# joeyz0z/ConZIC

Measured on AMD Instinct MI355X. Metric: captions/sec (L=10, K=200, seq order), higher is better.
Workload: dtype bf16

## Files before the change

conzic_amd/csrc/engine.hip:

```cpp
#include <algorithm>
#include <map>
#include <string>
#include <vector>
#include <cmath>
#include <cstddef>
#include <cstring>

#include "../../include/conzic_hip.h"
#include "kernels.h"
#include "bridge_hash.h"

namespace czc {
thread_local char g_err[512] = {0};
thread_local int g_gemm_family = 0;
}
using namespace czc;

namespace {

struct Tensor {
  float* p = nullptr;
  std::vector<int64_t> shape;
  size_t numel = 0;
};
// ... 70 lines not shown
  float* d_img_n = nullptr; int img_B = 0;
  float logit_scale_exp = 1.f;
  int* h_totals = nullptr;
  int last_BT = 0, last_B = 0, last_T = 0;
  int bert_prune = 1;
  int bert_pruned_idx = -1;
  const int32_t* bert_pruned_rows = nullptr;
  int bert_fuse_splitk_ln = 1;
  int share_prefix = 1;
  int dedup = 1;
  float* d_staged = nullptr; int staged_cap = 0, staged_n = 0;
  int pack_branches = 1;
  int pool_last_layer = 1;
  int share_layer0 = 1;
  int pool_last_qkv = 1;
  int fuse_ln = 1;
  int resid16 = 1;
  int fold_ln = 1;
  int prof = 0;
  std::map<std::string, ProfKind> pk;
  int64_t stat_clip_rows = 0, stat_clip_seqs = 0, stat_bert_rows = 0, stat_steps = 0;
  int64_t stat_refine_rows = 0, stat_refine_seqs = 0;
  int64_t stat_dedup_seqs = 0;
  czc_control_fn ctl_fn = nullptr; void* ctl_user = nullptr;
  int32_t* h_ctl_ids = nullptr; float* h_ctl_scores = nullptr; size_t h_ctl_cap = 0;
  int memo = 0;
  int64_t stat_memo_hits = 0, stat_memo_images = 0;
  int memo_rows = 0;
  int64_t stat_memo_row_hits = 0, stat_memo_row_steps = 0;
  int32_t* h_memo_list = nullptr; size_t h_memo_list_cap = 0;
// ... 128 lines not shown
    E_HIP(hipMemcpyAsync(l.qkv_b + 2 * H, vb, (size_t)H * 4, hipMemcpyDeviceToDevice, e->st));
    E_CHECK(need(e, o + ".weight", (size_t)H * H, &t)); E_CHECK(to_act(e, prec, t, (size_t)H * H, &l.o_w));
    E_CHECK(need(e, o + ".bias", H, &l.o_b));
    E_CHECK(need(e, ln1 + ".weight", H, &l.ln1_g)); E_CHECK(need(e, ln1 + ".bias", H, &l.ln1_b));
    E_CHECK(need(e, fc1 + ".weight", (size_t)I * H, &t)); E_CHECK(to_act(e, prec, t, (size_t)I * H, &l.fc1_w));
    E_CHECK(need(e, fc1 + ".bias", I, &l.fc1_b));
    E_CHECK(need(e, fc2 + ".weight", (size_t)H * I, &t)); E_CHECK(to_act(e, prec, t, (size_t)H * I, &l.fc2_w));
    E_CHECK(need(e, fc2 + ".bias", H, &l.fc2_b));
    E_CHECK(need(e, ln2 + ".weight", H, &l.ln2_g)); E_CHECK(need(e, ln2 + ".bias", H, &l.ln2_b));
  }
  return 0;
}

int gemm_ex(czc_engine* e, int prec, const char* kind, const GemmArgs& g) {
  ProfScope ps(e, kind, 2.0 * g.M * (double)g.N * g.K);
  E_CHECK(launch_gemm(prec, g, e->st));
  return 0;
}

int gemm(czc_engine* e, int prec, const char* kind, const void* A, int lda, const void* W, int ldw, const float* bias,
         const float* resid, int ldr, void* out_act, float* out_f32, int ldc, int M, int N, int K, int act) {
  GemmArgs g;
  g.A = A; g.lda = lda; g.W = W; g.ldw = ldw; g.bias = bias; g.resid = resid; g.ldr = ldr;
  g.out_act = out_act; g.out_f32 = out_f32; g.ldc = ldc; g.M = M; g.N = N; g.K = K; g.act = act;
  return gemm_ex(e, prec, kind, g);
}

int gemm_x16(czc_engine* e, int prec, const char* kind, const void* A, int lda, const void* W, const float* bias, void* x16, int M,
             int N, int K, float* part = nullptr, long part_ld = 0) {
  GemmArgs g;
  g.A = A; g.lda = lda; g.W = W; g.ldw = K; g.bias = bias; g.resid = (const float*)x16; g.ldr = N;
  g.out_act = nullptr; g.out_f32 = (float*)x16; g.ldc = N; g.M = M; g.N = N; g.K = K; g.act = ACT_NONE; g.x16 = 1;
  g.row_part = part; g.part_ld = part_ld;
// ... 30 lines not shown
  TowerPlan tp; const int* pool_idx = nullptr; int n_pool = 0; bool r16 = false; const float* ln_stat0 = nullptr; Layer0Rows l0;
};

int clip_stack(czc_engine* e, const StackDesc& d, float* x, float** pooled = nullptr) {
  const int P = d.P, M = d.M, H = d.H, I = d.I, heads = d.heads, max_keys = d.max_keys, n_pool = d.n_pool;
  const float eps = d.eps; const bool r16 = d.r16; const char* gk = d.gk; const size_t esz = prec_bytes(P);
  const SegTable& tab = d.tab; const TowerPlan& tp = d.tp; const Layer0Rows& l0 = d.l0; std::vector<LayerW>& L = *d.L;
  void *y, *qkv, *ctx, *hbuf;
  E_CHECK(ensure(e, "cs_y", (size_t)M * H * esz, &y));
  E_CHECK(ensure(e, "cs_qkv", (size_t)M * 3 * H * esz, &qkv));
  E_CHECK(ensure(e, "cs_ctx", (size_t)M * H * esz, &ctx));
  E_CHECK(ensure(e, "cs_h", (size_t)M * I * esz, &hbuf));
  const float scale = 1.0f / sqrtf(64.0f);
  const bool text = !strcmp(gk, "gemm_clip_text") || !strcmp(gk, "gemm_clip_refine");
  const char *ak = text ? "attention_clip_text" : "attention", *rk = text ? "rowops_clip_text" : "rowops";
  const double attn_flops = 4.0 * H * tp.pairs;
  const bool rowln = !r16 && prec_is_half(P) && e->fuse_ln && H == 512 && M >= g_rowln_min_m && I % 32 == 0;
  const bool fold = r16 && e->fold_ln && !L.empty() && L[0].qkv_wf && d.ln_stat0;
  float *part = nullptr, *stat = nullptr;
  if (fold) E_CHECK(ensure(e, "cs_part", (size_t)(H / 32) * M * 8, (void**)&part));
  if (fold) E_CHECK(ensure(e, "cs_stat", (size_t)M * 8 + 256, (void**)&stat));
  auto finalize = [&](int rows, int N, bool always = false) -> int {
    if (!always && gemm_wreg_stats_in_kernel(rows, N)) return 0;
    ProfScope ps(e, rk, 0);
    return launch_ln_finalize(part, M, H / 32, rows, eps, stat, e->st);
  };
  auto folded_gemm = [&](const void* Ax, const void* Wf, const float* bf, const float* st_, void* out, int rows, int N, int act, int ldc = 0) -> int {
    GemmArgs g;
    g.A = Ax; g.lda = H; g.W = Wf; g.ldw = H; g.bias = bf; g.resid = nullptr; g.ldr = 0; g.out_act = out; g.out_f32 = nullptr; g.ldc = ldc ? ldc : N;
    g.M = rows; g.N = N; g.K = H; g.act = act;
// ... 1009 lines not shown
    snprintf(czc::g_err, sizeof(czc::g_err), "czc_create: unknown precision");
    return CZC_ERR_ARG;
  }
  int ndev = 0;
  if (hipGetDeviceCount(&ndev) != hipSuccess || ndev <= 0) {
    snprintf(czc::g_err, sizeof(czc::g_err), "czc_create: no HIP device visible (the engine has no CPU fallback)");
    return CZC_ERR_HIP;
  }
  if (device_id < 0 || device_id >= ndev) {
    snprintf(czc::g_err, sizeof(czc::g_err), "czc_create: device %d out of range", device_id);
    return CZC_ERR_ARG;
  }
  czc_engine* e = new czc_engine();
  e->cfg = *cfg;
  e->dev = device_id;
  e->refine = cfg->precision == CZC_PREC_REFINE;
  e->pc = cfg->precision == CZC_PREC_F32 ? PREC_F32
          : (cfg->precision == CZC_PREC_SPLIT ? PREC_F16X3
             : ((cfg->precision == CZC_PREC_FP16 || e->refine) ? PREC_F16 : PREC_BF16));
  e->pb = cfg->precision == CZC_PREC_ALL_BF16 ? PREC_BF16
                                              : (cfg->precision == CZC_PREC_F32 ? PREC_F32 : PREC_F16X3);
  e->pv = e->refine ? (int)PREC_F16X3 : e->pc;
  e->esz = prec_bytes(e->pc);
  e->eb = prec_bytes(e->pb);
  if (hipSetDevice(device_id) != hipSuccess || hipStreamCreate(&e->st) != hipSuccess ||
      hipHostMalloc((void**)&e->h_totals, 256) != hipSuccess) {
    snprintf(czc::g_err, sizeof(czc::g_err), "czc_create: stream/host allocation failed");
    delete e;
    return CZC_ERR_HIP;
  }
// ... 30 lines not shown
int czc_replicate(czc_engine* p, czc_engine** out) {
  if (!p || !out) return CZC_ERR_ARG;
  if (!p->finalized) return fail(p, CZC_ERR_STATE, "czc_replicate: czc_finalize_weights first%s");
  czc_engine* e = new czc_engine();
  e->cfg = p->cfg; e->dev = p->dev; e->finalized = true; e->shares_weights = true;
  e->esz = p->esz; e->pb = p->pb; e->pc = p->pc; e->pv = p->pv; e->eb = p->eb;
  e->refine = p->refine; e->refine_theta_x = p->refine_theta_x; e->refine_samples = p->refine_samples; e->refine_samples_step = p->refine_samples_step;
  e->refine_guard_dev = p->refine_guard_dev; e->refine_gate_delta = p->refine_gate_delta; e->refine_theta_gen = p->refine_theta_gen;
  e->refine_rows16 = p->refine_rows16; e->refine_rows16_factor = p->refine_rows16_factor;
  e->memo = p->memo; e->memo_rows = p->memo_rows; e->fluency_chunk = p->fluency_chunk; e->regions_chunk = p->regions_chunk;
  e->w = p->w; e->bert = p->bert; e->ctext = p->ctext; e->cvis = p->cvis; e->ctext_x = p->ctext_x;
  e->mlm_dense_w = p->mlm_dense_w; e->decoder_w = p->decoder_w; e->tproj_w = p->tproj_w; e->vproj_w = p->vproj_w;
  e->patch_w = p->patch_w; e->tproj_wx = p->tproj_wx;
  e->logit_scale_exp = p->logit_scale_exp;
  e->share_prefix = p->share_prefix; e->dedup = p->dedup; e->pack_branches = p->pack_branches; e->pool_last_layer = p->pool_last_layer; e->pool_last_qkv = p->pool_last_qkv; e->share_layer0 = p->share_layer0;
  e->fuse_ln = p->fuse_ln; e->bert_prune = p->bert_prune; e->bert_fuse_splitk_ln = p->bert_fuse_splitk_ln; e->resid16 = p->resid16; e->fold_ln = p->fold_ln;
  memset(&e->bd, 0, sizeof(e->bd));
  if (hipSetDevice(e->dev) != hipSuccess || hipStreamCreate(&e->st) != hipSuccess ||
      hipHostMalloc((void**)&e->h_totals, 256) != hipSuccess) {
    e->w.clear();
    delete e;
    return fail(p, CZC_ERR_HIP, "czc_replicate: stream/host allocation failed%s");
  }
  *out = e;
  return CZC_OK;
}

int czc_load_tensor(czc_engine* e, const char* name, int dtype, int ndim, const int64_t* shape, const void* src) {
  if (e && e->shares_weights) return fail(e, CZC_ERR_STATE, "czc_load_tensor: a replica shares its parent's weights%s");
  if (!e || !name || !src || ndim < 0 || ndim > 8) return CZC_ERR_ARG;
// ... 1281 lines not shown
  e->ctl_fn = fn;
  e->ctl_user = fn ? user : nullptr;
  return CZC_OK;
}

int czc_set_option(czc_engine* e, const char* name, int value) {
  if (!e || !name) return CZC_ERR_ARG;
  if (!strcmp(name, "share_prefix")) { e->share_prefix = value ? 1 : 0; return CZC_OK; }
  if (!strcmp(name, "dedup")) { e->dedup = value ? 1 : 0; return CZC_OK; }
  if (!strcmp(name, "bert_prune")) { e->bert_prune = value ? 1 : 0; return CZC_OK; }
  if (!strcmp(name, "bert_fuse_splitk_ln")) { e->bert_fuse_splitk_ln = value ? 1 : 0; return CZC_OK; }
  if (!strcmp(name, "pack_branches")) { e->pack_branches = value ? 1 : 0; return CZC_OK; }
  if (!strcmp(name, "pool_last_layer")) { e->pool_last_layer = value ? 1 : 0; return CZC_OK; }
  if (!strcmp(name, "share_layer0")) { e->share_layer0 = value ? 1 : 0; return CZC_OK; }
  if (!strcmp(name, "pool_last_qkv")) { e->pool_last_qkv = value ? 1 : 0; return CZC_OK; }
  if (!strcmp(name, "fuse_ln")) { e->fuse_ln = value; return CZC_OK; }
  const auto fold_ready = [&]() -> int {
    if (e->finalized && wants_folded_ln(e) && (e->ctext.empty() || !e->ctext[0].qkv_wf))
      return fail(e, CZC_ERR_STATE, "option %s: this engine was finalized without the folded-LayerNorm operands (set it before czc_finalize_weights)", name);
    return CZC_OK;
  };
  if (!strcmp(name, "resid16")) { const int old = e->resid16; e->resid16 = value < 0 ? 0 : value; const int rc = fold_ready(); if (rc) e->resid16 = old; return rc; }
  if (!strcmp(name, "fold_ln")) { const int old = e->fold_ln; e->fold_ln = value ? 1 : 0; const int rc = fold_ready(); if (rc) e->fold_ln = old; return rc; }
  if (!strcmp(name, "refine_samples")) { e->refine_samples = value < 0 ? 0 : value; return CZC_OK; }
  if (!strcmp(name, "refine_samples_step")) { e->refine_samples_step = value < 0 ? 0 : value; return CZC_OK; }
  if (!strcmp(name, "refine_theta_x1000")) { e->refine_theta_x = (float)value / 1000.f; return CZC_OK; }
  if (!strcmp(name, "refine_theta_gen_x1000")) { e->refine_theta_gen = (float)value / 1000.f; return CZC_OK; }
  if (!strcmp(name, "refine_guard_x1e6")) { e->refine_guard_dev = (float)value * 1e-6f; return CZC_OK; }
  if (!strcmp(name, "refine_gate_x1e6")) { e->refine_gate_delta = value < 0 ? 0.f : (float)value * 1e-6f; return CZC_OK; }
  if (!strcmp(name, "refine_rows16")) { const int old = e->refine_rows16; e->refine_rows16 = value ? 1 : 0; const int rc = fold_ready(); if (rc) e->refine_rows16 = old; return rc; }
// ... 12 lines not shown
  if (!strcmp(name, "regions_chunk")) {
    if (value < 1 || value > CZC_MAX_REGIONS) return fail(e, CZC_ERR_ARG, "option %s: 1..1024", name);
    e->regions_chunk = value;
    return CZC_OK;
  }
  if (!strcmp(name, "refine_rows16_x1000")) { e->refine_rows16_factor = value < 1000 ? 1.f : (float)value / 1000.f; return CZC_OK; }
  return fail(e, CZC_ERR_ARG, "unknown option %s", name);
}

int czc_get_option(czc_engine* e, const char* name, int* value) {
  if (!e || !name || !value) return CZC_ERR_ARG;
  const bool r16 = e->refine && e->refine_rows16 && e->cfg.clip_hidden == 512;
  const float f16x = r16 ? e->refine_rows16_factor : 1.f;
  struct { const char* n; int v; } tab[] = {
      {"share_prefix", e->share_prefix}, {"bert_prune", e->bert_prune}, {"pack_branches", e->pack_branches},
      {"dedup", e->dedup}, {"pool_last_layer", e->pool_last_layer}, {"pool_last_qkv", e->pool_last_qkv}, {"share_layer0", e->share_layer0}, {"bert_fuse_splitk_ln", e->bert_fuse_splitk_ln}, {"fuse_ln", e->fuse_ln}, {"resid16", e->resid16}, {"fold_ln", e->fold_ln},
      {"refine_samples", e->refine_samples}, {"refine_samples_step", e->refine_samples_step}, {"refine_theta_x1000", (int)lrintf(e->refine_theta_x * 1000.f)},
      {"refine_theta_gen_x1000", (int)lrintf(e->refine_theta_gen * 1000.f)},
      {"refine_guard_x1e6", (int)lrintf(e->refine_guard_dev * 1e6f)}, {"refine_gate_x1e6", (int)lrintf(e->refine_gate_delta * 1e6f)},
      {"refine_rows16", e->refine_rows16}, {"memo", e->memo}, {"memo_rows", e->memo_rows}, {"index_groups", e->index_groups}, {"fluency_chunk", e->fluency_chunk}, {"regions_chunk", e->regions_chunk}, {"refine_rows16_x1000", (int)lrintf(e->refine_rows16_factor * 1000.f)},
      {"refine_guard_generate_x1e6", (int)lrintf(e->refine_guard_dev * f16x * 1e6f)},
      {"refine_gate_generate_x1e6", (int)lrintf(e->refine_gate_delta * f16x * 1e6f)},
      {"has_folded_ln_weights", !e->ctext.empty() && e->ctext[0].qkv_wf ? 1 : 0},
  };
  for (auto& t : tab) if (!strcmp(name, t.n)) { *value = t.v; return CZC_OK; }
  return fail(e, CZC_ERR_ARG, "unknown option %s", name);
}

int czc_sync(czc_engine* e) {
  if (!e) return CZC_ERR_ARG;
  E_HIP(hipSetDevice(e->dev));
// ... 162 lines not shown
```

conzic_amd/csrc/gemm256.hip:

```cpp
#include <type_traits>

#include "kernels.h"

namespace czc {

namespace {

constexpr int TM = 256, TN = 256;

template <int ACT>
__device__ __forceinline__ float act_fn(float v) {
  if (ACT == ACT_QUICK_GELU) return v * __builtin_amdgcn_rcpf(1.0f + __builtin_amdgcn_exp2f(-2.4554669595930156f * v));
  return v;
}

__device__ __forceinline__ void tile_of(int t, int tiles_m, int tiles_n, int& tm, int& tn) {
  const int nt = tiles_m * tiles_n;
  const int xcd = t & 7, q = nt >> 3, r = nt & 7;
  const int base = (xcd < r) ? xcd * (q + 1) : r * (q + 1) + (xcd - r) * q;
  const int lin = base + (t >> 3);
  tm = lin / tiles_n;
  tn = lin - tm * tiles_n;
}

// ... 337 lines not shown
          unsigned char* dst = oa + ((long)row * g.ldc + c8) * 4;
          *(h8*)dst = hh;
          *(h8*)(dst + 16) = ll;
        }
      }
    }
  }
}

__device__ __forceinline__ int tile_count(int tiles_m, int tiles_n) {
  const int grid = gridDim.x, wg = blockIdx.x, nt = tiles_m * tiles_n;
  return wg < nt ? (nt - 1 - wg) / grid + 1 : 0;
}
__device__ __forceinline__ void tile_at(int i, int tiles_m, int tiles_n, int& tm, int& tn) {
  tile_of(blockIdx.x + i * gridDim.x, tiles_m, tiles_n, tm, tn);
}

__device__ __forceinline__ void start_stagger(int stagger, int nt, int share) {
  if (!stagger) return;
  const int b = (int)blockIdx.x, tau = stagger & 255, bonus = stagger >> 8;
  const int rem = nt % (int)gridDim.x;
  unsigned long long dt = (unsigned long long)(((b >> 3) / share) & 7) * tau;
  if (rem && b >= rem) dt += bonus;
  dt *= 100ull;
  const unsigned long long t0 = __builtin_amdgcn_s_memrealtime();
  while (__builtin_amdgcn_s_memrealtime() - t0 < dt) __builtin_amdgcn_s_sleep(8);
}

constexpr int QROWB = 64;
constexpr int QA_BYTES = TM * QROWB;
// ... 113 lines not shown
      a0 = CZC_RA(1, 2);
      CZC_MM(c0, a1, 1, 0); CZC_MM(c1, a1, 1, 1);
      a1 = CZC_RA(1, 3);
      CZC_MM(c0, a0, 2, 0); CZC_MM(c1, a0, 2, 1);
      CZC_MM(c0, a1, 3, 0); CZC_MM(c1, a1, 3, 1);
#undef CZC_RA
#undef CZC_RB
#undef CZC_MM
    }
    tile_epilogue<ACT, OUT_F32, HT>(g, acc, smem + QS * QSTAGE + wave * 4096, m0, n0, wm, wn, lane);
  }
}



template <int ACT, bool OUT_F32, bool F16 = false, bool X16 = false>
__global__ __launch_bounds__(512) void gemm256x_kernel(GemmArgs g, int tiles_m, int tiles_n, int stagger) {
  using HT = std::conditional_t<F16, f16_t, bf16_t>;
  extern __shared__ __attribute__((aligned(16))) unsigned char smem[];
  const int tid = threadIdx.x;
  const int lane = tid & 63;
  const int wave = __builtin_amdgcn_readfirstlane(tid >> 6);
  const int nk = g.K >> 5;
  const int lda_b = g.lda * 2, ldw_b = g.ldw * 2;
  start_stagger(stagger, tiles_m * tiles_n, tiles_n);
  const int my_tiles = tile_count(tiles_m, tiles_n);
  const int total = my_tiles * nk;

  const unsigned lds0 = __builtin_amdgcn_readfirstlane(
      (unsigned)(unsigned long long)(__attribute__((address_space(3))) unsigned char*)smem);
  const int rbase = wave * 32 + (lane >> 2);
  const int cq = ((lane & 3) ^ ((lane >> 4) & 3)) << 4;
  const int a0 = rbase * lda_b + cq, w0 = rbase * ldw_b + cq;
  const int a16 = 16 * lda_b, w16 = 16 * ldw_b;
  u32x4_t rsA, rsW;
  rsA.x = rsA.y = rsA.z = 0; rsA.w = 0x00020000u;
  rsW = rsA;
  int is = 0, is_ti = 0, is_kt = 0;
  auto issue_rebase = [&]() {
    int tm, tn;
    tile_at(is_ti, tiles_m, tiles_n, tm, tn);
    const int m0 = tm * TM, n0 = tn * TN;
    const unsigned long long pa = (unsigned long long)g.A + (unsigned long long)m0 * lda_b;
    const unsigned long long pw = (unsigned long long)g.W + (unsigned long long)n0 * ldw_b;
    rsA.x = (unsigned)pa; rsA.y = (unsigned)(pa >> 32) & 0xffffu; rsA.z = (unsigned)(min(TM, g.M - m0) * lda_b);
    rsW.x = (unsigned)pw; rsW.y = (unsigned)(pw >> 32) & 0xffffu; rsW.z = (unsigned)(min(TN, g.N - n0) * ldw_b);
  };
  auto issue_next = [&]() {
    const unsigned dstA = lds0 + (is & (QS - 1)) * QSTAGE + wave * (32 * QROWB);
    const unsigned dstW = dstA + QA_BYTES;
    const unsigned so = is_kt * QROWB;
    unsigned keep;
    asm volatile(
        "s_mov_b32 %0, m0\n\t"
        "s_mov_b32 m0, %1\n\ts_nop 0\n\tbuffer_load_dwordx4 %3, %7, %9 offen lds\n\t"
        "s_add_u32 m0, m0, 0x400\n\ts_nop 0\n\tbuffer_load_dwordx4 %4, %7, %9 offen lds\n\t"
// ... 18 lines not shown
    for (int s = 0; s < AHEAD && s < total; ++s) issue_next();
    {
      const int later = (total < AHEAD ? total : AHEAD) - 1;
      if (later >= 2) asm volatile("s_waitcnt vmcnt(8)" ::: "memory");
      else if (later == 1) asm volatile("s_waitcnt vmcnt(4)" ::: "memory");
      else asm volatile("s_waitcnt vmcnt(0)" ::: "memory");
    }
    __builtin_amdgcn_s_barrier();
    asm volatile("" ::: "memory");

    const int wn = wave & 3;
    const int half = lane >> 5;
    const int arow = GRP * 128 + (lane & 31);
    const int brow = wn * 64 + (lane & 31);
    int step = 0;
    const int steady_end = total - 3;
    for (int ti = 0; ti < my_tiles; ++ti) {
      int tm, tn;
      tile_at(ti, tiles_m, tiles_n, tm, tn);
      const int m0 = tm * TM, n0 = tn * TN;
      f32x16_t acc[4][2];
#pragma unroll
      for (int i = 0; i < 4; ++i)
#pragma unroll
        for (int j = 0; j < 2; ++j)
#pragma unroll
          for (int r = 0; r < 16; ++r) acc[i][j][r] = 0.f;
      if (GRP) {
        __builtin_amdgcn_s_barrier();
        asm volatile("" ::: "memory");
      }
      auto kstep = [&](auto steady_c) __attribute__((always_inline)) {
        constexpr bool STEADY = decltype(steady_c)::value;
        const unsigned char* sA = smem + (step & (QS - 1)) * QSTAGE;
        const unsigned char* sB = sA + QA_BYTES;
        if (STEADY || step + AHEAD < total) issue_next();
        uint4 fa[2][4], fb[2][2];
#pragma unroll
        for (int ks = 0; ks < 2; ++ks) {
#pragma unroll
          for (int j = 0; j < 2; ++j) fb[ks][j] = *(const uint4*)(sB + swzq(brow + 32 * j, 2 * ks + half));
#pragma unroll
          for (int i = 0; i < 4; ++i) fa[ks][i] = *(const uint4*)(sA + swzq(arow + 32 * i, 2 * ks + half));
        }
        if (GRP) {
          if (STEADY || step + 3 < total) asm volatile("s_waitcnt vmcnt(8)" ::: "memory");
          else if (step + 2 < total) asm volatile("s_waitcnt vmcnt(4)" ::: "memory");
          else asm volatile("s_waitcnt vmcnt(0)" ::: "memory");
        }
        __builtin_amdgcn_sched_barrier(0);
        __builtin_amdgcn_s_barrier();
        asm volatile("" ::: "memory");
        __builtin_amdgcn_s_setprio(1);
#pragma unroll
        for (int ks = 0; ks < 2; ++ks)
#pragma unroll
          for (int i = 0; i < 4; ++i)
#pragma unroll
            for (int j = 0; j < 2; ++j) acc[i][j] = Half<HT>::mfma(fb[ks][j], fa[ks][i], acc[i][j]);
        __builtin_amdgcn_s_setprio(0);
        __builtin_amdgcn_sched_barrier(0);
        if (!GRP) {
          if (STEADY || step + 2 < total) asm volatile("s_waitcnt vmcnt(4)" ::: "memory");
          else asm volatile("s_waitcnt vmcnt(0)" ::: "memory");
        }
        __builtin_amdgcn_s_barrier();
        asm volatile("" ::: "memory");
      };
      int kt = 0;
      for (; kt < nk && step < steady_end; ++kt, ++step) kstep(std::true_type());
      for (; kt < nk; ++kt, ++step) kstep(std::false_type());
      if (!GRP) {
        __builtin_amdgcn_s_barrier();
        asm volatile("" ::: "memory");
      }
      unsigned char* patch = smem + QS * QSTAGE + wave * 4096;
      if constexpr (X16) {
        tile_epilogue_x16_asm<2>(g, acc, patch, m0, n0, GRP, wn * 64, lane);
      } else if constexpr (OUT_F32 && ACT == ACT_NONE) {
        if (g.resid && g.out_f32 && !g.out_act) tile_epilogue_f32_asm<2>(g, acc, patch, m0, n0, GRP, wn * 64, lane);
        else tile_epilogue<ACT, OUT_F32, HT>(g, acc, patch, m0, n0, GRP, wn, lane);
      } else {
        tile_epilogue<ACT, OUT_F32, HT>(g, acc, patch, m0, n0, GRP, wn, lane);
      }
    }
  };
  if (wave >> 2) run(std::integral_constant<int, 1>());
  else run(std::integral_constant<int, 0>());
}

template <int ACT, bool OUT_F32>
__global__ __launch_bounds__(768) void gemm256sq_kernel(GemmArgs g, int tiles_m, int tiles_n) {
  extern __shared__ __attribute__((aligned(16))) unsigned char smem[];
  const int tid = threadIdx.x;
  const int lane = tid & 63;
  const int wave = __builtin_amdgcn_readfirstlane(tid >> 6);
  const int nk = g.K >> 4;
  const int lda_b = g.lda * 4, ldw_b = g.ldw * 4;
  const int my_tiles = tile_count(tiles_m, tiles_n);
// ... 418 lines not shown
}

int launch_gemm256(const GemmArgs& g, hipStream_t st) {
  constexpr int shp = QS * QSTAGE + 8 * 4096;
  static PerDeviceInit per_dev;
  const LaunchInit init = per_dev.get([](LaunchInit&) -> int {
#define CZC_ATTR(K_) CZC_HIP_CHECK(hipFuncSetAttribute((const void*)K_, hipFuncAttributeMaxDynamicSharedMemorySize, shp))
#define CZC_ATTR4(K_) CZC_ATTR((K_<ACT_NONE, false, false>)); CZC_ATTR((K_<ACT_NONE, true, false>)); \
                      CZC_ATTR((K_<ACT_QUICK_GELU, false, false>)); CZC_ATTR((K_<ACT_QUICK_GELU, true, false>)); \
                      CZC_ATTR((K_<ACT_NONE, false, true>)); CZC_ATTR((K_<ACT_NONE, true, true>)); \
                      CZC_ATTR((K_<ACT_QUICK_GELU, false, true>)); CZC_ATTR((K_<ACT_QUICK_GELU, true, true>))
    CZC_ATTR4(gemm256q_kernel);
    CZC_ATTR4(gemm256x_kernel);
    CZC_ATTR((gemm256x_kernel<ACT_NONE, true, false, true>));
    CZC_ATTR((gemm256x_kernel<ACT_NONE, true, true, true>));
#undef CZC_ATTR4
#undef CZC_ATTR
    return 0;
  });
  if (init.rc) return launch_init_failed("gemm256");
  const int n_cu = init.n_cu;
  const int tiles_m = cdiv(g.M, TM), tiles_n = cdiv(g.N, TN);
  const bool f32 = g.out_f32 != nullptr || g.resid != nullptr;
  dim3 gq(tiles_m * tiles_n < n_cu ? tiles_m * tiles_n : n_cu);
  const bool pp = g_use_gemm256 == 5 || (g_use_gemm256 != 3 && f32);
  g_gemm_family = (g.x16 || pp) ? GF_RING_PINGPONG : GF_RING_LOADER;
#define CZC_GO(K_, A_, F_, H_, T_, ...) hipLaunchKernelGGL((K_<A_, F_, H_>), gq, dim3(T_), shp, st, g, tiles_m, tiles_n, ##__VA_ARGS__)
#define CZC_DISPATCH(K_, T_, ...)                                                                                          \
  do {                                                                                                                     \
    if (g.f16) {                                                                                                           \
      if (g.act == ACT_QUICK_GELU) { if (f32) CZC_GO(K_, ACT_QUICK_GELU, true, true, T_, ##__VA_ARGS__); else CZC_GO(K_, ACT_QUICK_GELU, false, true, T_, ##__VA_ARGS__); } \
      else { if (f32) CZC_GO(K_, ACT_NONE, true, true, T_, ##__VA_ARGS__); else CZC_GO(K_, ACT_NONE, false, true, T_, ##__VA_ARGS__); }                               \
    } else {                                                                                                               \
      if (g.act == ACT_QUICK_GELU) { if (f32) CZC_GO(K_, ACT_QUICK_GELU, true, false, T_, ##__VA_ARGS__); else CZC_GO(K_, ACT_QUICK_GELU, false, false, T_, ##__VA_ARGS__); } \
      else { if (f32) CZC_GO(K_, ACT_NONE, true, false, T_, ##__VA_ARGS__); else CZC_GO(K_, ACT_NONE, false, false, T_, ##__VA_ARGS__); }                             \
    }                                                                                                                      \
  } while (0)
  const int stagger256 = (f32 && tiles_m * tiles_n / (int)gq.x >= 4) ? (2 | 32 << 8) : 0;
  if (g.x16) {
    if (g.f16) hipLaunchKernelGGL((gemm256x_kernel<ACT_NONE, true, true, true>), gq, dim3(512), shp, st, g, tiles_m, tiles_n, stagger256);
    else hipLaunchKernelGGL((gemm256x_kernel<ACT_NONE, true, false, true>), gq, dim3(512), shp, st, g, tiles_m, tiles_n, stagger256);
  } else if (pp) CZC_DISPATCH(gemm256x_kernel, 512, stagger256);
  else CZC_DISPATCH(gemm256q_kernel, 768);
#undef CZC_DISPATCH
#undef CZC_GO
  CZC_HIP_CHECK(hipGetLastError());
  return 0;
}

int g_use_gemm256s = 1;
int g_gemm256s_min_m = 16384;

bool gemm256s_eligible(const GemmArgs& g) {
  return g_use_gemm256s && g.M >= g_gemm256s_min_m && g.N % 8 == 0 && g.K % 32 == 0 && g.ldc % 8 == 0 && g.lda % 8 == 0 && g.ldw % 8 == 0 &&
// ... 31 lines not shown
```

conzic_amd/csrc/kernels.h:

```cpp
#pragma once
#include <vector>

#include "common.h"

namespace czc {

struct GemmArgs {
  const void* A = nullptr; int lda = 0;
  const void* W = nullptr; int ldw = 0;
  const float* bias = nullptr;
  const float* resid = nullptr; int ldr = 0;
  void* out_act = nullptr; float* out_f32 = nullptr; int ldc = 0;
  int M = 0, N = 0, K = 0;
  int act = 0;
  int f16 = 0;
  int x16 = 0;
  float* row_part = nullptr;
  long part_ld = 0;
  const float* ln_stat = nullptr;
  const float* ln_part = nullptr;
  long ln_part_ld = 0;
  const float* ln_gamma = nullptr;
  const float* ln_beta = nullptr;
  float ln_eps = 0.f;
  struct SplitkPending* splitk_pending = nullptr;
};
struct SplitkPending { const float* slabs = nullptr; int nslab = 0; long slab_stride = 0; int ld = 0; };
enum GemmFamily {
  GF_NONE = 0, GF_TILED_VEC = 1, GF_TILED_SCALAR = 2, GF_SPLITK = 3, GF_SKINNY = 4, GF_RING_LOADER = 5, GF_RING_PINGPONG = 6,
  GF_RING_SPLIT = 7, GF_WREG = 8, GF_WREG_LNF = 9, GF_WREG_RESID = 10, GF_ROWLN = 11
};
int launch_gemm(int prec, const GemmArgs& g, hipStream_t st);
bool gemm256_eligible(const GemmArgs& g);
int launch_gemm256(const GemmArgs& g, hipStream_t st);
extern int g_use_gemm256;
bool gemm256s_eligible(const GemmArgs& g);
int launch_gemm256s(const GemmArgs& g, hipStream_t st);
extern int g_use_gemm256s, g_gemm256s_min_m;
bool gemm_rowln_eligible(const GemmArgs& g);
int launch_gemm_rowln(const GemmArgs& g, hipStream_t st);
// ... 218 lines not shown
int launch_refine_finish(const int* own_off, const int* own_len, const int* count, const int* count_off, const int* kr_dev, int B, int K,
                         int* pre_off, int* eos_idx, hipStream_t st);

int launch_normalize_split(const float* src, long n, int D, split_t* dst, int* bad, int bad_stride, hipStream_t st);
int index_scan_groups(int n, int D, int k, int groups);
int launch_index_search(const split_t* index, int n, int D, const split_t* queries, int Q, int k, int G,
                        unsigned long long* part, int* out_ids, float* out_cos, hipStream_t st);

int fluency_expand_tables(int R, int seed_len, int Lmax, const int32_t* len_of_row, int32_t* row_of_seq, int32_t* col_of_seq);
int launch_expand_mask_rows(const int* rows, int T, const int* row_of_seq, const int* col_of_seq, int N, int mask_id, int* ids_out,
                            int* target, int* gen_rows, hipStream_t st);
int launch_logprob_target(const float* logits, int N, int V, const int* target, float temperature, const int* out_idx, float* logp,
                          int* rank, int* nonfinite, hipStream_t st);
int launch_pll_sum(const float* logp, int R, int Lmax, const int* len_of_row, float* pll, hipStream_t st);

constexpr int HOOKS_ABI = 0x060e;
struct Hooks {
  char* (*err_buf)();
  decltype(&launch_gemm) gemm;
  decltype(&launch_gemm_rowln) gemm_rowln;
  decltype(&launch_layernorm) layernorm;
  decltype(&launch_convert) convert;
  decltype(&launch_act_to_f32) act_to_f32;
  decltype(&launch_attention) attention;
  decltype(&launch_attention_shared) attention_shared;
  decltype(&launch_attention_shared_split) attention_shared_split;
  decltype(&launch_softmax_mask_topk) softmax_mask_topk;
  decltype(&launch_bridge_precompute) bridge_precompute;
  decltype(&launch_bridge) bridge;
  decltype(&launch_l2_normalize) l2_normalize;
  decltype(&launch_combine) combine;
// ... 59 lines not shown
```

conzic_amd/native.py:

```python
from __future__ import annotations

import ctypes as C
import os
from typing import Optional

_HERE = os.path.dirname(os.path.abspath(__file__))
LIB_PATH = os.environ.get("CZC_LIB_PATH") or os.path.join(_HERE, "lib", "libconzic_hip.so")
HEADER_PATH = os.path.join(os.path.dirname(_HERE), "include", "conzic_hip.h")
TEST_LIB_PATH = os.environ.get("CZC_TEST_LIB_PATH") or (LIB_PATH[:-3] + "_test.so" if LIB_PATH.endswith(".so")
                                                        else os.path.join(os.path.dirname(LIB_PATH), "libconzic_hip_test.so"))
TEST_HEADER_PATH = os.path.join(os.path.dirname(_HERE), "include", "conzic_hip_test.h")

PREC_BF16 = 0
PREC_F32 = 1
PREC_ALL_BF16 = 2
PREC_SPLIT = 3
PREC_FP16 = 4
PREC_REFINE = 5
CLIP_MAX_LEN = 77
MAX_BERT_LEN = 64
MAX_VOCAB_SETS = 4096
MAX_TOPK = 1024
MAX_RIVALS = 16
MAX_REGIONS = 1024
# ... 114 lines not shown
    "czc_memo_stats": (_I, [_P, C.POINTER(C.c_int64), C.POINTER(C.c_int64)]),
    "czc_memo_rows_stats": (_I, [_P, C.POINTER(C.c_int64), C.POINTER(C.c_int64)]),
}
PRIVATE_SIGNATURES = {"czc_internal_hooks": (_P, [_I])}


class GemmLayout(C.Structure):
    _fields_ = ([(n, C.c_int32) for n in ("precision", "form", "M", "N", "K", "act", "lda", "ldw", "ldc", "ldr", "c0", "flags",
                                          "part_ld")] + [("eps", C.c_float)] +
                [(n, C.c_void_p) for n in ("A", "W", "bias", "resid", "gamma", "beta", "ln_part", "out_f32", "out_act", "part_out")])


TEST_SIGNATURES = {
    "czc_test_gemm": (_I, [_I, _I, _I, _I, _P, _P, _P, _P, _I, _P]),
    "czc_test_gemm_x16": (_I, [_I, _I, _I, _I, _P, _P, _P, _P, _P, _P]),
    "czc_test_ln_fold_gemm": (_I, [_I, _I, _I, _P, _P, _P, _P, _P, _P, C.c_float, _I, _P, _P]),
    "czc_test_layernorm_x16": (_I, [_I, _I, _P, _P, _P, C.c_float, _P]),
    "czc_test_gemm_rowln": (_I, [_I, _I, _I, _P, _P, _P, _P, _P, _P, C.c_float, _P, _P]),
    "czc_bench_gemm": (_I, [_I, _I, _I, _I, _I, _I, _I, _I, C.POINTER(C.c_double)]),
    "czc_test_set_option": (_I, [C.c_char_p, _I]),
    "czc_test_layernorm": (_I, [_I, _I, _I, _P, _P, _P, C.c_float, _P]),
    "czc_test_attention": (_I, [_I, _I, _P, _I, _I, C.c_float, _P, _P]),
    "czc_test_attention_plan": (_I, [_I, _I, _I, _I, _I, C.c_float, _P, _P, _I, _P, _P]),
    "czc_test_attention_pooled": (_I, [_I, _I, _I, _I, C.c_float, _P, _P, _P, _P, _P, _P]),
    "czc_test_attention_seq": (_I, [_I, _I, _P, _I, _I, _I, _I, C.c_float, _P, _P]),
    "czc_test_attention_mapped": (_I, [_I, _I, _I, _I, C.c_float, _P, _P, _P, _I, _P, _P]),
    "czc_test_layer0_plan": (_I, [_I, _I, _P, _P, _I, _P, _P, _P, _P, _I, _P, _I, _P]),
    "czc_test_text_tower": (_I, [_P, _I, _I, _P, _P, _P, _P]),
    "czc_test_topk": (_I, [_I, _I, _I, _P, _P, C.c_float, _I, _I, _P, _P, _P]),
    "czc_test_bridge": (_I, [C.POINTER(BridgeTables), C.POINTER(Config), _I, _I, _P, _P, _P]),
# ... 80 lines not shown
```

Measured before the change: 83.40.

## Add dynamic atomic tile scheduling to persistent 256x GEMM for text tower

Adds a DYN variant of the persistent gemm256x kernel in which blocks pull output tiles from per-slot atomic counters instead of a static strided assignment. The next tile index is prefetched with an in-loop global atomic issued by wave 0. Counters come from a pooled device buffer that is reset once per CLIP text/refine stack pass. The aim is to balance load across CUs when the tile count exceeds the grid. In exchange it adds atomics, extra LDS traffic and a memset per pass, and it relies on inline asm for exec-masking and waitcnt handling.

```diff
diff --git a/conzic_amd/csrc/engine.hip b/conzic_amd/csrc/engine.hip
--- a/conzic_amd/csrc/engine.hip
+++ b/conzic_amd/csrc/engine.hip
@@ -5,6 +5,7 @@
 #include <cmath>
 #include <cstddef>
 #include <cstring>
+#include <cstdlib>
 
 #include "../../include/conzic_hip.h"
 #include "kernels.h"
@@ -108,6 +109,9 @@
   int pool_last_layer = 1;
   int share_layer0 = 1;
   int pool_last_qkv = 1;
+  int dyn_tiles = 1;
+  DynCounters dyn;
+  bool dyn_pass = false;
   int fuse_ln = 1;
   int resid16 = 1;
   int fold_ln = 1;
@@ -266,9 +270,34 @@
 
 int gemm_ex(czc_engine* e, int prec, const char* kind, const GemmArgs& g) {
   ProfScope ps(e, kind, 2.0 * g.M * (double)g.N * g.K);
+  if (e->dyn_pass && !g.dyn_ctr) {
+    GemmArgs gd = g;
+    gd.dyn_ctr = e->dyn.take();
+    E_CHECK(launch_gemm(prec, gd, e->st));
+    return 0;
+  }
   E_CHECK(launch_gemm(prec, g, e->st));
   return 0;
 }
+
+constexpr int DYN_POOL_BLOCKS = 256;
+struct DynPass {
+  czc_engine* e;
+  explicit DynPass(czc_engine* e_) : e(e_) {}
+  int open() {
+    if (!e->dyn_tiles) return 0;
+    void* p;
+    E_CHECK(ensure(e, "cs_dyn", (size_t)DYN_POOL_BLOCKS * DYN_CTR_INTS * 4, &p));
+    if (e->dyn.base != (int*)p) {
+      E_HIP(hipMemsetAsync(p, 0, (size_t)DYN_POOL_BLOCKS * DYN_CTR_INTS * 4, e->st));
+      e->dyn.base = (int*)p; e->dyn.n_blocks = DYN_POOL_BLOCKS; e->dyn.next = 0;
+    }
+    E_HIP(e->dyn.reset(e->st));
+    e->dyn_pass = true;
+    return 0;
+  }
+  ~DynPass() { e->dyn_pass = false; }
+};
 
 int gemm(czc_engine* e, int prec, const char* kind, const void* A, int lda, const void* W, int ldw, const float* bias,
          const float* resid, int ldr, void* out_act, float* out_f32, int ldc, int M, int N, int K, int act) {
@@ -329,6 +358,8 @@
   const float scale = 1.0f / sqrtf(64.0f);
   const bool text = !strcmp(gk, "gemm_clip_text") || !strcmp(gk, "gemm_clip_refine");
   const char *ak = text ? "attention_clip_text" : "attention", *rk = text ? "rowops_clip_text" : "rowops";
+  DynPass dyn_pass(e);
+  if (text) E_CHECK(dyn_pass.open());
   const double attn_flops = 4.0 * H * tp.pairs;
   const bool rowln = !r16 && prec_is_half(P) && e->fuse_ln && H == 512 && M >= g_rowln_min_m && I % 32 == 0;
   const bool fold = r16 && e->fold_ln && !L.empty() && L[0].qkv_wf && d.ln_stat0;
@@ -1368,6 +1399,7 @@
   czc_engine* e = new czc_engine();
   e->cfg = *cfg;
   e->dev = device_id;
+  if (const char* v = getenv("CZC_DYN_TILES")) e->dyn_tiles = atoi(v) ? 1 : 0;
   e->refine = cfg->precision == CZC_PREC_REFINE;
   e->pc = cfg->precision == CZC_PREC_F32 ? PREC_F32
           : (cfg->precision == CZC_PREC_SPLIT ? PREC_F16X3
@@ -1428,6 +1460,7 @@
   e->patch_w = p->patch_w; e->tproj_wx = p->tproj_wx;
   e->logit_scale_exp = p->logit_scale_exp;
   e->share_prefix = p->share_prefix; e->dedup = p->dedup; e->pack_branches = p->pack_branches; e->pool_last_layer = p->pool_last_layer; e->pool_last_qkv = p->pool_last_qkv; e->share_layer0 = p->share_layer0;
+  e->dyn_tiles = p->dyn_tiles;
   e->fuse_ln = p->fuse_ln; e->bert_prune = p->bert_prune; e->bert_fuse_splitk_ln = p->bert_fuse_splitk_ln; e->resid16 = p->resid16; e->fold_ln = p->fold_ln;
   memset(&e->bd, 0, sizeof(e->bd));
   if (hipSetDevice(e->dev) != hipSuccess || hipStreamCreate(&e->st) != hipSuccess ||
@@ -2739,6 +2772,7 @@
   if (!strcmp(name, "pool_last_layer")) { e->pool_last_layer = value ? 1 : 0; return CZC_OK; }
   if (!strcmp(name, "share_layer0")) { e->share_layer0 = value ? 1 : 0; return CZC_OK; }
   if (!strcmp(name, "pool_last_qkv")) { e->pool_last_qkv = value ? 1 : 0; return CZC_OK; }
+  if (!strcmp(name, "dyn_tiles")) { e->dyn_tiles = value ? 1 : 0; return CZC_OK; }
   if (!strcmp(name, "fuse_ln")) { e->fuse_ln = value; return CZC_OK; }
   const auto fold_ready = [&]() -> int {
     if (e->finalized && wants_folded_ln(e) && (e->ctext.empty() || !e->ctext[0].qkv_wf))
@@ -2781,7 +2815,7 @@
   const float f16x = r16 ? e->refine_rows16_factor : 1.f;
   struct { const char* n; int v; } tab[] = {
       {"share_prefix", e->share_prefix}, {"bert_prune", e->bert_prune}, {"pack_branches", e->pack_branches},
-      {"dedup", e->dedup}, {"pool_last_layer", e->pool_last_layer}, {"pool_last_qkv", e->pool_last_qkv}, {"share_layer0", e->share_layer0}, {"bert_fuse_splitk_ln", e->bert_fuse_splitk_ln}, {"fuse_ln", e->fuse_ln}, {"resid16", e->resid16}, {"fold_ln", e->fold_ln},
+      {"dedup", e->dedup}, {"pool_last_layer", e->pool_last_layer}, {"pool_last_qkv", e->pool_last_qkv}, {"share_layer0", e->share_layer0}, {"bert_fuse_splitk_ln", e->bert_fuse_splitk_ln}, {"fuse_ln", e->fuse_ln}, {"dyn_tiles", e->dyn_tiles}, {"resid16", e->resid16}, {"fold_ln", e->fold_ln},
       {"refine_samples", e->refine_samples}, {"refine_samples_step", e->refine_samples_step}, {"refine_theta_x1000", (int)lrintf(e->refine_theta_x * 1000.f)},
       {"refine_theta_gen_x1000", (int)lrintf(e->refine_theta_gen * 1000.f)},
       {"refine_guard_x1e6", (int)lrintf(e->refine_guard_dev * 1e6f)}, {"refine_gate_x1e6", (int)lrintf(e->refine_gate_delta * 1e6f)},
diff --git a/conzic_amd/csrc/gemm256.hip b/conzic_amd/csrc/gemm256.hip
--- a/conzic_amd/csrc/gemm256.hip
+++ b/conzic_amd/csrc/gemm256.hip
@@ -375,6 +375,12 @@
 }
 __device__ __forceinline__ void tile_at(int i, int tiles_m, int tiles_n, int& tm, int& tn) {
   tile_of(blockIdx.x + i * gridDim.x, tiles_m, tiles_n, tm, tn);
+}
+
+__device__ __forceinline__ void slot_share(int slot, int nt, int& base, int& size) {
+  const int q = nt >> 3, r = nt & 7;
+  base = (slot < r) ? slot * (q + 1) : r * (q + 1) + (slot - r) * q;
+  size = q + (slot < r ? 1 : 0);
 }
 
 __device__ __forceinline__ void start_stagger(int stagger, int nt, int share) {
@@ -518,7 +524,7 @@
 
 
 
-template <int ACT, bool OUT_F32, bool F16 = false, bool X16 = false>
+template <int ACT, bool OUT_F32, bool F16 = false, bool X16 = false, bool DYN = false>
 __global__ __launch_bounds__(512) void gemm256x_kernel(GemmArgs g, int tiles_m, int tiles_n, int stagger) {
   using HT = std::conditional_t<F16, f16_t, bf16_t>;
   extern __shared__ __attribute__((aligned(16))) unsigned char smem[];
@@ -527,9 +533,28 @@
   const int wave = __builtin_amdgcn_readfirstlane(tid >> 6);
   const int nk = g.K >> 5;
   const int lda_b = g.lda * 2, ldw_b = g.ldw * 2;
-  start_stagger(stagger, tiles_m * tiles_n, tiles_n);
-  const int my_tiles = tile_count(tiles_m, tiles_n);
-  const int total = my_tiles * nk;
+  int* const dyn_ctr = DYN ? g.dyn_ctr + (blockIdx.x & 7) * 8 : nullptr;
+  __attribute__((address_space(3))) volatile int* const dyn_box = (__attribute__((address_space(3))) volatile int*)(smem + QS * QSTAGE);
+  int dyn_base = 0, dyn_size = 0, cur_lin = -1, nxt_lin = -1;
+  if constexpr (DYN) {
+    slot_share(blockIdx.x & 7, tiles_m * tiles_n, dyn_base, dyn_size);
+    if (tid == 0) {
+      const int k0 = __hip_atomic_fetch_add(dyn_ctr, 1, __ATOMIC_RELAXED, __HIP_MEMORY_SCOPE_AGENT);
+      const int k1 = __hip_atomic_fetch_add(dyn_ctr, 1, __ATOMIC_RELAXED, __HIP_MEMORY_SCOPE_AGENT);
+      dyn_box[0] = k0 < dyn_size ? dyn_base + k0 : -1;
+      dyn_box[1] = k1 < dyn_size ? dyn_base + k1 : -1;
+    }
+    __syncthreads();
+    cur_lin = __builtin_amdgcn_readfirstlane(dyn_box[0]);
+    nxt_lin = __builtin_amdgcn_readfirstlane(dyn_box[1]);
+    if (cur_lin < 0) return;
+    start_stagger(stagger & 255, tiles_m * tiles_n, tiles_n);
+  } else {
+    start_stagger(stagger, tiles_m * tiles_n, tiles_n);
+  }
+  const int my_tiles = DYN ? 0 : tile_count(tiles_m, tiles_n);
+  int total = DYN ? (nxt_lin >= 0 ? 2 : 1) * nk : my_tiles * nk;
+  int reb_lin = cur_lin;
 
   const unsigned lds0 = __builtin_amdgcn_readfirstlane(
       (unsigned)(unsigned long long)(__attribute__((address_space(3))) unsigned char*)smem);
@@ -543,7 +568,8 @@
   int is = 0, is_ti = 0, is_kt = 0;
   auto issue_rebase = [&]() {
     int tm, tn;
-    tile_at(is_ti, tiles_m, tiles_n, tm, tn);
+    if constexpr (DYN) { tm = reb_lin / tiles_n; tn = reb_lin - tm * tiles_n; }
+    else tile_at(is_ti, tiles_m, tiles_n, tm, tn);
     const int m0 = tm * TM, n0 = tn * TN;
     const unsigned long long pa = (unsigned long long)g.A + (unsigned long long)m0 * lda_b;
     const unsigned long long pw = (unsigned long long)g.W + (unsigned long long)n0 * ldw_b;
@@ -592,10 +618,17 @@
     const int arow = GRP * 128 + (lane & 31);
     const int brow = wn * 64 + (lane & 31);
     int step = 0;
-    const int steady_end = total - 3;
-    for (int ti = 0; ti < my_tiles; ++ti) {
+    int steady_end = total - 3;
+    for (int ti = 0; DYN ? cur_lin >= 0 : ti < my_tiles; ++ti) {
       int tm, tn;
-      tile_at(ti, tiles_m, tiles_n, tm, tn);
+      if constexpr (DYN) {
+        tm = cur_lin / tiles_n; tn = cur_lin - tm * tiles_n;
+        reb_lin = nxt_lin;
+        total = (ti + (nxt_lin >= 0 ? 2 : 1)) * nk;
+        steady_end = total - 3;
+      } else {
+        tile_at(ti, tiles_m, tiles_n, tm, tn);
+      }
       const int m0 = tm * TM, n0 = tn * TN;
       f32x16_t acc[4][2];
 #pragma unroll
@@ -608,10 +641,21 @@
         __builtin_amdgcn_s_barrier();
         asm volatile("" ::: "memory");
       }
-      auto kstep = [&](auto steady_c) __attribute__((always_inline)) {
+      auto kstep = [&](auto steady_c, auto pull_c) __attribute__((always_inline)) {
         constexpr bool STEADY = decltype(steady_c)::value;
+        constexpr bool PULL = decltype(pull_c)::value && !GRP;
         const unsigned char* sA = smem + (step & (QS - 1)) * QSTAGE;
         const unsigned char* sB = sA + QA_BYTES;
+        int pulled = 0;
+        if constexpr (PULL) {
+          const unsigned em = __builtin_amdgcn_readfirstlane(wave == 0 ? 1u : 0u);
+          const unsigned long long cp = (unsigned long long)dyn_ctr;
+          unsigned long long keep;
+          asm volatile("s_mov_b64 %1, exec\n\ts_mov_b32 exec_lo, %2\n\ts_mov_b32 exec_hi, 0\n\tglobal_atomic_add %0, %3, %4, off sc0\n\ts_mov_b64 exec, %1"
+                       : "=&v"(pulled), "=&s"(keep)
+                       : "s"(em), "v"(cp), "v"(1)
+                       : "memory");
+        }
         if (STEADY || step + AHEAD < total) issue_next();
         uint4 fa[2][4], fb[2][2];
 #pragma unroll
@@ -642,12 +686,25 @@
           if (STEADY || step + 2 < total) asm volatile("s_waitcnt vmcnt(4)" ::: "memory");
           else asm volatile("s_waitcnt vmcnt(0)" ::: "memory");
         }
+        if constexpr (PULL) {
+          asm volatile("s_waitcnt vmcnt(4)" : "+v"(pulled) : : "memory");
+          if (tid == 0) dyn_box[2] = pulled < dyn_size ? dyn_base + pulled : -1;
+          asm volatile("s_waitcnt lgkmcnt(0)" ::: "memory");
+        }
         __builtin_amdgcn_s_barrier();
         asm volatile("" ::: "memory");
       };
       int kt = 0;
-      for (; kt < nk && step < steady_end; ++kt, ++step) kstep(std::true_type());
-      for (; kt < nk; ++kt, ++step) kstep(std::false_type());
+      int nn_lin = -1;
+      if constexpr (DYN) {
+        if (nxt_lin >= 0) {
+          kstep(std::false_type(), std::true_type());
+          ++kt, ++step;
+          nn_lin = __builtin_amdgcn_readfirstlane(dyn_box[2]);
+        }
+      }
+      for (; kt < nk && step < steady_end; ++kt, ++step) kstep(std::true_type(), std::false_type());
+      for (; kt < nk; ++kt, ++step) kstep(std::false_type(), std::false_type());
       if (!GRP) {
         __builtin_amdgcn_s_barrier();
         asm volatile("" ::: "memory");
@@ -661,6 +718,7 @@
       } else {
         tile_epilogue<ACT, OUT_F32, HT>(g, acc, patch, m0, n0, GRP, wn, lane);
       }
+      if constexpr (DYN) { cur_lin = nxt_lin; nxt_lin = nn_lin; }
     }
   };
   if (wave >> 2) run(std::integral_constant<int, 1>());
@@ -1109,6 +1167,10 @@
     CZC_ATTR4(gemm256x_kernel);
     CZC_ATTR((gemm256x_kernel<ACT_NONE, true, false, true>));
     CZC_ATTR((gemm256x_kernel<ACT_NONE, true, true, true>));
+    CZC_ATTR((gemm256x_kernel<ACT_NONE, true, false, true, true>));
+    CZC_ATTR((gemm256x_kernel<ACT_NONE, true, true, true, true>));
+    CZC_ATTR((gemm256x_kernel<ACT_NONE, true, false, false, true>));
+    CZC_ATTR((gemm256x_kernel<ACT_NONE, true, true, false, true>));
 #undef CZC_ATTR4
 #undef CZC_ATTR
     return 0;
@@ -1132,7 +1194,14 @@
     }                                                                                                                      \
   } while (0)
   const int stagger256 = (f32 && tiles_m * tiles_n / (int)gq.x >= 4) ? (2 | 32 << 8) : 0;
-  if (g.x16) {
+  const bool dyn = g.dyn_ctr && g.K >= 128 && tiles_m * tiles_n > (int)gq.x && (g.x16 || (pp && f32 && g.act == ACT_NONE));
+  if (dyn && g.x16) {
+    if (g.f16) hipLaunchKernelGGL((gemm256x_kernel<ACT_NONE, true, true, true, true>), gq, dim3(512), shp, st, g, tiles_m, tiles_n, stagger256);
+    else hipLaunchKernelGGL((gemm256x_kernel<ACT_NONE, true, false, true, true>), gq, dim3(512), shp, st, g, tiles_m, tiles_n, stagger256);
+  } else if (dyn) {
+    if (g.f16) hipLaunchKernelGGL((gemm256x_kernel<ACT_NONE, true, true, false, true>), gq, dim3(512), shp, st, g, tiles_m, tiles_n, stagger256);
+    else hipLaunchKernelGGL((gemm256x_kernel<ACT_NONE, true, false, false, true>), gq, dim3(512), shp, st, g, tiles_m, tiles_n, stagger256);
+  } else if (g.x16) {
     if (g.f16) hipLaunchKernelGGL((gemm256x_kernel<ACT_NONE, true, true, true>), gq, dim3(512), shp, st, g, tiles_m, tiles_n, stagger256);
     else hipLaunchKernelGGL((gemm256x_kernel<ACT_NONE, true, false, true>), gq, dim3(512), shp, st, g, tiles_m, tiles_n, stagger256);
   } else if (pp) CZC_DISPATCH(gemm256x_kernel, 512, stagger256);
diff --git a/conzic_amd/csrc/kernels.h b/conzic_amd/csrc/kernels.h
--- a/conzic_amd/csrc/kernels.h
+++ b/conzic_amd/csrc/kernels.h
@@ -24,6 +24,18 @@
   const float* ln_beta = nullptr;
   float ln_eps = 0.f;
   struct SplitkPending* splitk_pending = nullptr;
+  int* dyn_ctr = nullptr;
+};
+constexpr int DYN_CTR_INTS = 64;
+struct DynCounters {
+  int* base = nullptr; int n_blocks = 0, next = 0;
+  int* take() { return next < n_blocks ? base + (size_t)DYN_CTR_INTS * next++ : nullptr; }
+  hipError_t reset(hipStream_t st) {
+    if (!base || !next) return hipSuccess;
+    const size_t used = (size_t)next * DYN_CTR_INTS * 4;
+    next = 0;
+    return hipMemsetAsync(base, 0, used, st);
+  }
 };
 struct SplitkPending { const float* slabs = nullptr; int nslab = 0; long slab_stride = 0; int ld = 0; };
 enum GemmFamily {
@@ -272,7 +284,7 @@
                           int* rank, int* nonfinite, hipStream_t st);
 int launch_pll_sum(const float* logp, int R, int Lmax, const int* len_of_row, float* pll, hipStream_t st);
 
-constexpr int HOOKS_ABI = 0x060e;
+constexpr int HOOKS_ABI = 0x060f;
 struct Hooks {
   char* (*err_buf)();
   decltype(&launch_gemm) gemm;
diff --git a/conzic_amd/native.py b/conzic_amd/native.py
--- a/conzic_amd/native.py
+++ b/conzic_amd/native.py
@@ -152,6 +152,7 @@
 TEST_SIGNATURES = {
     "czc_test_gemm": (_I, [_I, _I, _I, _I, _P, _P, _P, _P, _I, _P]),
     "czc_test_gemm_x16": (_I, [_I, _I, _I, _I, _P, _P, _P, _P, _P, _P]),
+    "czc_test_gemm_x16_series": (_I, [_I, _I, _I, _I, _P, _P, _P, _P, _I, _I, _I, _P, _P, _P]),
     "czc_test_ln_fold_gemm": (_I, [_I, _I, _I, _P, _P, _P, _P, _P, _P, C.c_float, _I, _P, _P]),
     "czc_test_layernorm_x16": (_I, [_I, _I, _P, _P, _P, C.c_float, _P]),
     "czc_test_gemm_rowln": (_I, [_I, _I, _I, _P, _P, _P, _P, _P, _P, C.c_float, _P, _P]),
```

New measurement: 83.30 (median of 2 runs). No clear change (-0.1%).
